# beautifulv0id/Convex-2D-GPU-Collision-Detection

Hardware: AMD Instinct MI355X
Metric: sat_pair_tests_per_s (higher is better)
Workload: dtype f32

## Files before the change

convex-2d-gpu-collision-detection_amd/csrc/c2d_mc_poly.hip:

```cpp
#include <type_traits>

#include "c2d_internal.hpp"
#include "c2d_math.hpp"

#ifdef C2D_MC_STATS
namespace c2d {
__device__ unsigned long long c2d_mc_poly_stats_words[12];
}
#define C2D_MC_STAT(i, v)                                                                                     \
    do {                                                                                                      \
        const unsigned long long v__ = (unsigned long long)(v);                                               \
        if ((threadIdx.x & 63) == 0 && v__) atomicAdd(&c2d::c2d_mc_poly_stats_words[i], v__);                 \
    } while (0)
#endif
#include "c2d_mc_core.hpp"

namespace c2d {

#ifndef C2D_MC_POLY_PLAIN_PAIR_LOOP
#define C2D_MC_POLY_PLAIN_PAIR_LOOP 0
#endif
constexpr int KM = C2D_POLY_KMAX;
#ifndef C2D_MC_POLY_IN_PLACE
#define C2D_MC_POLY_IN_PLACE 48
#endif
#ifndef C2D_MC_POLY_SURV_SLOTS
#define C2D_MC_POLY_SURV_SLOTS ((64 + C2D_MC_POLY_IN_PLACE + 15) / 16 * 16)
#endif
constexpr int kSurvSlots = C2D_MC_POLY_SURV_SLOTS;
static_assert(63 + C2D_MC_POLY_IN_PLACE - 1 < kSurvSlots, "survivor queue too small for a full push");

struct PolyScene {
    float sx, sy, st, sw, sh;
    uint32_t x0;
    bool use_x0;
    int ka, kb;
    C2D_DEV bool tame() const { return use_x0 || x0 != 0u; }
};

struct PolyQueue {
    float4 axis[KM];
    float4 pre[KM];
    float4 ctr[KM];
    float2 rvert[KM];
    float2 overt[KM];
    float4 surv_a[kSurvSlots];
    float2 surv_b[kSurvSlots];
    uint32_t n_surv;
    SampleQueues sq;
};

C2D_DEV float wave_max(float v)
{
#pragma unroll
    for (int off = 32; off > 0; off >>= 1) v = __builtin_fmaxf(v, __shfl_xor(v, off, 64));
    return v;
}

C2D_DEV float lane_pick(const float (&a)[KM], uint32_t l)
{
    float v = a[0];
#pragma unroll
    for (int k = 1; k < KM; k++) v = l == (uint32_t)k ? a[k] : v;
    return v;
}

C2D_DEV PolyScene build_poly_scene(float rvx, float rvy, int ka, float px, float py, float theta, float ovx, float ovy, int kb, const StdDev& sd,
                                   PolyQueue& q)
{
    const uint32_t lane = threadIdx.x & 63, l = lane & 15;
    PolyScene sc;
    sc.sx = sd.x; sc.sy = sd.y; sc.st = sd.theta; sc.sw = sd.width; sc.sh = sd.height;
    sc.ka = ka; sc.kb = kb;
    const float rx0 = __shfl(rvx, 0, 64), ry0 = __shfl(rvy, 0, 64), ox0 = __shfl(ovx, 0, 64), oy0 = __shfl(ovy, 0, 64);
    const float rxl = (int)l < ka ? rvx : rx0, ryl = (int)l < ka ? rvy : ry0;
    const float oxl = (int)l < kb ? ovx : ox0, oyl = (int)l < kb ? ovy : oy0;
    float s, c;
    sincos_(theta, s, c);
    const float wx = dot2(c, rxl, -s, ryl) + px, wy = dot2(s, rxl, c, ryl) + py;
    wave_lds_sync();
    if (lane < KM) {
        q.rvert[l] = make_float2(wx, wy);
        q.overt[l] = make_float2(oxl, oyl);
    }
    if (lane == 0) q.n_surv = 0;
    wave_lds_sync();
    const float2 v1 = q.rvert[(l + 1) & 15];
    const float nx = -(v1.y - wy), ny = v1.x - wx;
    float rmin = 0.0f, rmax = 0.0f, p_first = 0.0f;
#pragma unroll
    for (int k = 0; k < KM; k++) {
        const float2 v = q.rvert[k];
        const float p = nx * v.x + ny * v.y;
        if (k == 0) { rmin = rmax = p_first = p; }
        else { rmin = __builtin_fminf(rmin, p); rmax = __builtin_fmaxf(rmax, p); }
    }
    const float fxm = 1.0f + kNormalMax * __builtin_fabsf(sc.sw), fym = 1.0f + kNormalMax * __builtin_fabsf(sc.sh);
    const float ex = fxm * oxl, ey = fym * oyl;
    const float rho = wave_max(__builtin_sqrtf(ex * ex + ey * ey)) * (1.0f + 0x1p-10f);
    const float D = kNormalMax * (__builtin_fabsf(sc.sx) + __builtin_fabsf(sc.sy));
    const float n2 = __builtin_sqrtf(nx * nx + ny * ny), n1 = __builtin_fabsf(nx) + __builtin_fabsf(ny);
    const float M = (n2 * rho) * (1.0f + 0x1p-10f) + 0x1p-12f * (n1 * (rho + D));
    const float hi = rmax + M, lo = rmin - M;
    float phi = hi + 0x1p-20f * __builtin_fabsf(hi), plo = lo - 0x1p-20f * __builtin_fabsf(lo);
    const bool real_edge = (int)l < ka && n1 > 0.0f;
    if (!real_edge) { phi = __builtin_inff(); plo = -__builtin_inff(); }
    float r0 = 0.0f;
    {
        const float gx = nx * sc.sx, gy = ny * sc.sy;
        const float G = __builtin_sqrtf(gx * gx + gy * gy) * (1.0f + 0x1p-10f);
        const float L = plo > 0.0f ? plo : (phi < 0.0f ? -phi : 0.0f);
        if (real_edge && L > 0.0f && G > 0.0f && L < 1e30f) r0 = L / G;
    }
    const float R0 = wave_max(r0);
    if (lane < KM) {
        q.axis[l] = make_float4(nx, ny, rmin, rmax);
        q.pre[l] = make_float4(plo, phi, p_first, 0.0f);
        q.ctr[l] = make_float4(nx, ny, plo, phi);
    }
    wave_lds_sync();
    auto below = [](float v, float bound) { return __builtin_fabsf(v) < bound; };
    auto length = [](float v) { const float a = __builtin_fabsf(v); return a < 1e8f && (a == 0.0f || a >= 1e-15f); };
    const float rel = 1e4f, ang = 1e15f;
    const bool mine = ((int)l >= ka || (length(rvx) && length(rvy))) && ((int)l >= kb || (length(ovx) && length(ovy)));
    const bool tame = __builtin_amdgcn_ballot_w64(!mine) == 0ull && length(px) && length(py) && below(theta, ang) && length(sd.x) && length(sd.y) &&
                      below(sd.theta, ang) && below(sd.width, rel) && below(sd.height, rel);
    sc.use_x0 = false;
    sc.x0 = 0xffffffffu;
    if (!tame) {
        sc.x0 = 0u;
        return sc;
    }
    radius_word_threshold(R0, sc.x0, sc.use_x0);
    return sc;
}

template <bool NANS>
C2D_DEV float min3_(float a, float b, float c)
{
    if constexpr (NANS) return __builtin_fminf(__builtin_fminf(a, b), c);
    float r;
    asm("v_min3_f32 %0, %1, %2, %3" : "=v"(r) : "v"(a), "v"(b), "v"(c));
    return r;
}
template <bool NANS>
C2D_DEV float max3_(float a, float b, float c)
{
    if constexpr (NANS) return __builtin_fmaxf(__builtin_fmaxf(a, b), c);
    float r;
    asm("v_max3_f32 %0, %1, %2, %3" : "=v"(r) : "v"(a), "v"(b), "v"(c));
    return r;
}

template <int CB>
C2D_DEV void poly_sampled_vertices(const PolyQueue& q, float dx, float dy, float c, float s, float fx, float fy, float (&ox)[CB], float (&oy)[CB])
{
#pragma unroll
    for (int k = 0; k < CB; k++) {
        const float2 b = q.overt[k];
        const float x = fx * b.x, y = fy * b.y;
        ox[k] = dot2(c, x, -s, y) + dx;
        oy[k] = dot2(s, x, c, y) + dy;
    }
}

template <int CB, bool NANS>
C2D_DEV unsigned long long poly_stage_robot(const PolyScene& sc, const PolyQueue& q, const float (&ox)[CB], const float (&oy)[CB], unsigned long long lanes)
{
    unsigned long long sep = 0ull;
    const int ka = sc.ka;
#pragma nounroll
    for (int i = 0; i < ka; i++) {
        const float4 A = q.axis[i];
        float p0 = A.x * ox[0] + A.y * oy[0];
        float omin = p0, omax = p0;
#pragma unroll
        for (int k = 1; k < CB; k++) {
            const float p = A.x * ox[k] + A.y * oy[k];
            omin = __builtin_fminf(omin, p);
            omax = __builtin_fmaxf(omax, p);
        }
        unsigned long long m = __builtin_amdgcn_ballot_w64(A.w < omin) | __builtin_amdgcn_ballot_w64(omax < A.z);
        if constexpr (NANS) m &= __builtin_amdgcn_ballot_w64(first_projections_ordered(q.pre[i].z, p0));
        sep |= m;
    }
    return lanes & ~sep;
}

template <int CB, bool NANS>
C2D_DEV unsigned long long poly_stage_obstacle(const PolyScene& sc, const PolyQueue& q, const float (&ox)[CB], const float (&oy)[CB], unsigned long long lanes)
{
    unsigned long long sep = 0ull;
    const int ka = sc.ka;
    auto group = [&](auto g_const, auto j0_const) {
        constexpr int G = decltype(g_const)::value, j0 = decltype(j0_const)::value;
        float nx[G], ny[G], mn1[G], mx1[G], mn2[G], mx2[G], q0[G], r0[G];
#pragma unroll
        for (int a = 0; a < G; a++) {
            const int j = j0 + a, j1 = (j + 1) % CB;
            nx[a] = -(oy[j1] - oy[j]);
            ny[a] = ox[j1] - ox[j];
            q0[a] = nx[a] * ox[0] + ny[a] * oy[0];
            mn2[a] = mx2[a] = q0[a];
        }
#pragma unroll
        for (int k = 1; k < CB; k++) {
#pragma unroll
            for (int a = 0; a < G; a++) {
                const float p = nx[a] * ox[k] + ny[a] * oy[k];
                mn2[a] = __builtin_fminf(mn2[a], p);
                mx2[a] = __builtin_fmaxf(mx2[a], p);
            }
        }
        const float4* rv2 = reinterpret_cast<const float4*>(q.rvert);
        const int pairs = (ka + 1) >> 1;
#if C2D_MC_POLY_PLAIN_PAIR_LOOP
        float4 cur = rv2[0];
#else
        float4 cur = rv2[0];
        float4 nxt = rv2[pairs > 1 ? 1 : 0];
#endif
#pragma unroll
        for (int a = 0; a < G; a++) {
            r0[a] = nx[a] * cur.x + ny[a] * cur.y;
            const float p1 = nx[a] * cur.z + ny[a] * cur.w;
            mn1[a] = __builtin_fminf(r0[a], p1);
            mx1[a] = __builtin_fmaxf(r0[a], p1);
        }
#pragma nounroll
        for (int j = 1; j < pairs; j++) {
#if C2D_MC_POLY_PLAIN_PAIR_LOOP
            cur = rv2[j];
#else
            cur = nxt;
            nxt = rv2[j + 1 < pairs ? j + 1 : j];
#endif
#pragma unroll
            for (int a = 0; a < G; a++) {
                const float p0 = nx[a] * cur.x + ny[a] * cur.y, p1 = nx[a] * cur.z + ny[a] * cur.w;
                mn1[a] = min3_<NANS>(mn1[a], p0, p1);
                mx1[a] = max3_<NANS>(mx1[a], p0, p1);
            }
        }
#pragma unroll
        for (int a = 0; a < G; a++) {
            unsigned long long m = __builtin_amdgcn_ballot_w64(mx1[a] < mn2[a]) | __builtin_amdgcn_ballot_w64(mx2[a] < mn1[a]);
            if constexpr (NANS) m &= __builtin_amdgcn_ballot_w64(first_projections_ordered(r0[a], q0[a]));
            sep |= m;
        }
    };
    using std::integral_constant;
    if constexpr (CB >= 4) { group(integral_constant<int, 4>{}, integral_constant<int, 0>{}); if ((lanes & ~sep) == 0ull) return 0ull; }
    if constexpr (CB >= 8) { group(integral_constant<int, 4>{}, integral_constant<int, 4>{}); if ((lanes & ~sep) == 0ull) return 0ull; }
    if constexpr (CB >= 12) { group(integral_constant<int, 4>{}, integral_constant<int, 8>{}); if ((lanes & ~sep) == 0ull) return 0ull; }
    if constexpr (CB >= 16) { group(integral_constant<int, 4>{}, integral_constant<int, 12>{}); if ((lanes & ~sep) == 0ull) return 0ull; }
    if constexpr (CB % 4 != 0) group(integral_constant<int, CB % 4>{}, integral_constant<int, CB - CB % 4>{});
    return lanes & ~sep;
}

template <int CB, bool NANS, int STAGE>
C2D_DEV unsigned long long poly_sample_stage(const PolyScene& sc, const PolyQueue& q, float dx, float dy, float c, float s, float fx, float fy,
                                             unsigned long long lanes, bool& final)
{
    float ox[CB], oy[CB];
    poly_sampled_vertices<CB>(q, dx, dy, c, s, fx, fy, ox, oy);
    unsigned long long alive = lanes;
    final = true;
    if constexpr (STAGE != 2) {
        alive = poly_stage_robot<CB, NANS>(sc, q, ox, oy, alive);
        if (alive == 0ull) return 0ull;
    }
    if constexpr (STAGE == 1) {
        if (__popcll(alive) < C2D_MC_POLY_IN_PLACE) { final = false; return alive; }
        C2D_MC_STAT(8, __popcll(alive));
    }
    return poly_stage_obstacle<CB, NANS>(sc, q, ox, oy, alive);
}

template <bool NANS, int STAGE>
C2D_DEV unsigned long long poly_sample_stage_any(const PolyScene& sc, const PolyQueue& q, float dx, float dy, float c, float s, float fx, float fy,
                                                 unsigned long long lanes, bool& final)
{
#ifndef C2D_MC_POLY_EVEN_SLOTS
#define C2D_MC_POLY_EVEN_SLOTS 0
#endif
#define C2D_POLY_STAGE(CB) return poly_sample_stage<CB, NANS, STAGE>(sc, q, dx, dy, c, s, fx, fy, lanes, final)
    if constexpr (NANS || C2D_MC_POLY_EVEN_SLOTS) {
        switch ((sc.kb + 1) >> 1) {
        case 1: C2D_POLY_STAGE(2);
        case 2: C2D_POLY_STAGE(4);
        case 3: C2D_POLY_STAGE(6);
        case 4: C2D_POLY_STAGE(8);
        case 5: C2D_POLY_STAGE(10);
        case 6: C2D_POLY_STAGE(12);
        case 7: C2D_POLY_STAGE(14);
        default: C2D_POLY_STAGE(16);
        }
    } else {
        switch (sc.kb) {
        case 1: C2D_POLY_STAGE(1);
        case 2: C2D_POLY_STAGE(2);
        case 3: C2D_POLY_STAGE(3);
        case 4: C2D_POLY_STAGE(4);
        case 5: C2D_POLY_STAGE(5);
        case 6: C2D_POLY_STAGE(6);
        case 7: C2D_POLY_STAGE(7);
        case 8: C2D_POLY_STAGE(8);
        case 9: C2D_POLY_STAGE(9);
        case 10: C2D_POLY_STAGE(10);
        case 11: C2D_POLY_STAGE(11);
        case 12: C2D_POLY_STAGE(12);
        case 13: C2D_POLY_STAGE(13);
        case 14: C2D_POLY_STAGE(14);
        case 15: C2D_POLY_STAGE(15);
        default: C2D_POLY_STAGE(16);
        }
    }
#undef C2D_POLY_STAGE
}

C2D_DEV void poly_sample_shape(const PolyScene& sc, uint32_t radius_word, uint32_t angle_word, uint64_t seed, uint64_t scene_id, uint64_t sample, float& c,
                               float& s, float& fx, float& fy)
{
    float n2, n3;
    box_muller(radius_word, angle_word, n2, n3);
    const float dt = n2 * sc.st;
    const float dw = n3 * sc.sw;
    float dh = 0.0f;
    if (sc.sh != 0.0f) {
        const U4 b = philox_draw_block(seed, scene_id, sample >> 2, 4u + ((uint32_t)(sample >> 1) & 1u));
        const bool odd = (sample & 1) != 0;
        float n4, unused;
        box_muller(odd ? b.z : b.x, odd ? b.w : b.y, n4, unused);
        dh = n4 * sc.sh;
    }
    fx = 1.0f + dw;
    fy = 1.0f + dh;
    sincos_(dt, s, c);
}

struct PolyPolicy {
    using Scene = PolyScene;
    using Queue = PolyQueue;
    static C2D_DEV bool centre_pretest(const Scene& sc, const Queue& q, float dx, float dy, unsigned long long& miss_m)
    {
        bool miss = false;
#pragma nounroll
        for (int i = 0; i < sc.ka; i++) {
            const float4 A = q.ctr[i];
            const float t = fma_(A.x, dx, A.y * dy);
            miss |= (t > A.w) | (t < A.z);
        }
        miss_m = __builtin_amdgcn_ballot_w64(miss);
        return miss;
    }
    static C2D_DEV uint32_t evaluate_survivors(const Scene& sc, Queue& q, uint32_t& n, uint32_t take)
    {
        const uint32_t lane = threadIdx.x & 63;
        wave_lds_sync();
        const unsigned long long live_m = take >= 64 ? ~0ull : (1ull << take) - 1;
        const uint32_t src = n - take + (lane < take ? lane : 0);
        const float4 a = q.surv_a[src];
        const float2 b = q.surv_b[src];
        wave_lds_sync();
        n -= take;
        bool final;
        C2D_MC_STAT(9, take);
        return (uint32_t)__popcll(poly_sample_stage_any<false, 2>(sc, q, a.x, a.y, a.z, a.w, b.x, b.y, live_m, final));
    }
    static C2D_DEV uint32_t evaluate(const Scene& sc, Queue& q, uint32_t w2r, uint32_t w2a, float dx, float dy, uint64_t seed, uint64_t scene_id, uint64_t sample,
                                     unsigned long long live_m)
    {
        float c, s, fx, fy;
        poly_sample_shape(sc, w2r, w2a, seed, scene_id, sample, c, s, fx, fy);
        bool final;
        C2D_MC_STAT(5, __popcll(live_m));
        const unsigned long long alive = poly_sample_stage_any<false, 1>(sc, q, dx, dy, c, s, fx, fy, live_m, final);
        if (final) return (uint32_t)__popcll(alive);
        C2D_MC_STAT(6, __popcll(alive));
        uint32_t n = q.n_surv;
        if ((alive >> (threadIdx.x & 63)) & 1ull) {
            const uint32_t slot = n + __builtin_amdgcn_mbcnt_hi((uint32_t)(alive >> 32), __builtin_amdgcn_mbcnt_lo((uint32_t)alive, 0u));
            q.surv_a[slot] = make_float4(dx, dy, c, s);
            q.surv_b[slot] = make_float2(fx, fy);
        }
        n += (uint32_t)__popcll(alive);
        uint32_t hits = 0;
        if (n >= 64) hits = evaluate_survivors(sc, q, n, 64);
        wave_lds_sync();
        if ((threadIdx.x & 63) == 0) q.n_surv = n;
        wave_lds_sync();
        return hits;
    }
    static C2D_DEV uint32_t finish(const Scene& sc, Queue& q)
    {
        uint32_t n = q.n_surv;
        if (n == 0) return 0u;
        uint32_t hits = 0;
        while (n) hits += evaluate_survivors(sc, q, n, n < 64 ? n : 64u);
        wave_lds_sync();
        if ((threadIdx.x & 63) == 0) q.n_surv = 0;
        wave_lds_sync();
        return hits;
    }
    static C2D_DEV uint32_t plain(const Scene& sc, uint64_t seed, uint64_t scene_id, uint64_t begin, uint32_t count, const Queue& q)
    {
        const uint32_t lane = threadIdx.x & 63;
        uint32_t hits = 0;
#pragma nounroll
        for (uint32_t i = 0; i < count; i += 64) {
            const uint32_t left = count - i;
            const unsigned long long live_m = left >= 64 ? ~0ull : (1ull << left) - 1;
            const uint64_t sm = begin + i + lane;
            const uint32_t j = (uint32_t)sm & 3u;
            const U4 b0 = philox_draw_block(seed, scene_id, sm >> 2, 0), b1 = philox_draw_block(seed, scene_id, sm >> 2, 1);
            const U4 b2 = philox_draw_block(seed, scene_id, sm >> 2, 2u + (j >> 1));
            float dx, dy, c, s, fx, fy;
            sample_centre(sc, u4_word(b0, (int)j), u4_word(b1, (int)j), dx, dy);
            poly_sample_shape(sc, (j & 1u) ? b2.z : b2.x, (j & 1u) ? b2.w : b2.y, seed, scene_id, sm, c, s, fx, fy);
            bool final;
            hits += (uint32_t)__popcll(poly_sample_stage_any<true, 0>(sc, q, dx, dy, c, s, fx, fy, live_m, final));
        }
        return hits;
    }
};

struct PolyPairArgs {
    c2d_polygon robot, obstacle;
    float px, py, theta;
    StdDev sd;
    uint64_t seed, scene_id, sample_begin, n_samples;
    uint32_t chunk;
};

#ifndef C2D_MC_POLY_WAVES
#define C2D_MC_POLY_WAVES 5
#endif
#ifdef C2D_MC_CLOCK
C2D_MC_CLOCK_WORDS(c2d_mc_clock_poly_pair);
C2D_MC_CLOCK_WORDS(c2d_mc_clock_poly);
#endif
__global__ __launch_bounds__(kMcBlock, C2D_MC_POLY_WAVES) void mc_poly_pair_kernel(PolyPairArgs A, unsigned long long* __restrict__ d_hits)
{
    __shared__ PolyQueue s_queue[kWavesPerBlock];
    const uint32_t wave = __builtin_amdgcn_readfirstlane(threadIdx.x >> 6);
    const uint32_t l = threadIdx.x & 15;
    const PolyScene sc = build_poly_scene(lane_pick(A.robot.x, l), lane_pick(A.robot.y, l), (int)A.robot.k, A.px, A.py, A.theta, lane_pick(A.obstacle.x, l),
                                          lane_pick(A.obstacle.y, l), (int)A.obstacle.k, A.sd, s_queue[wave]);
    const uint64_t n_chunks = (A.n_samples + A.chunk - 1) / A.chunk;
    unsigned long long total = 0;
    C2D_MC_CLOCK_START();
    for (uint64_t ch = (uint64_t)blockIdx.x * kWavesPerBlock + wave; ch < n_chunks; ch += (uint64_t)gridDim.x * kWavesPerBlock) {
        const uint64_t off = ch * A.chunk;
        const uint64_t left = A.n_samples - off;
        const uint32_t count = left < A.chunk ? (uint32_t)left : A.chunk;
        total += wave_count_hits<PolyPolicy>(sc, A.seed, A.scene_id, A.sample_begin + off, count, s_queue[wave]);
    }
    C2D_MC_CLOCK_STOP(c2d_mc_clock_poly_pair);
    if ((threadIdx.x & 63) == 0 && total) atomicAdd(d_hits, total);
}

struct PolyScenesArgs {
    const StdDev* std_devs;
    const PositionWithVarAndPoseIdx* scenes;
    AdaptiveState* state;
    uint32_t* lists[2];
    uint32_t num_std_devs;
    uint64_t seed, scene_id_base;
    ScheduleArgs sched;
    uint32_t* hits;
    uint32_t burst_steps;
    uint32_t n_bins;
    float bins[16], acc[16];
    uint32_t* n_used;
    PoseCPVarAndPoseIdx* rows;
    const c2d_poly_pose* poly_poses;
    uint32_t num_poly_poses;
    c2d_polygon robot;
    uint32_t* async_err;
};

struct PolyBuilder {
    using Args = PolyScenesArgs;
    using Policy = PolyPolicy;
#ifdef C2D_MC_CLOCK
    static C2D_DEV unsigned long long* clock_words() { return c2d_mc_clock_poly; }
#endif
    static C2D_DEV PolyScene scene(const Args& A, const PositionWithVarAndPoseIdx& row, PolyQueue& q)
    {
        uint32_t pi = (uint32_t)(int)row.pose_idx, vi = (uint32_t)(int)row.var_idx;
        pi = pi < A.num_poly_poses ? pi : A.num_poly_poses - 1;
        vi = vi < A.num_std_devs ? vi : A.num_std_devs - 1;
        const c2d_poly_pose* pp = A.poly_poses + pi;
        const uint32_t l = threadIdx.x & 15;
        const float theta = pp->theta, ovx = pp->obstacle.x[l], ovy = pp->obstacle.y[l];
        uint32_t kb = pp->obstacle.k, ka = A.robot.k;
        if (kb < 1 || kb > (uint32_t)KM) {
            if ((threadIdx.x & 63) == 0) __hip_atomic_fetch_or(A.async_err, C2D_ASYNC_ERR_POLY_K, __ATOMIC_RELAXED, __HIP_MEMORY_SCOPE_SYSTEM);
            kb = kb < 1 ? 1u : (uint32_t)KM;
        }
        ka = ka < 1 ? 1u : (ka > (uint32_t)KM ? (uint32_t)KM : ka);
        return build_poly_scene(lane_pick(A.robot.x, l), lane_pick(A.robot.y, l), (int)ka, row.x, row.y, theta, ovx, ovy, (int)kb, A.std_devs[vi], q);
    }
};

template <bool BURST>
__global__ __launch_bounds__(kMcBlock, C2D_MC_POLY_WAVES) void mc_poly_scenes_advance_kernel(PolyScenesArgs A) { mc_scenes_advance_body<BURST, PolyBuilder>(A); }

}

using namespace c2d;

namespace {

const char* polygon_fault(const c2d_polygon* p)
{
    if (!p) return "NULL polygon";
    if (p->k < 1 || p->k > (uint32_t)C2D_POLY_KMAX) return "polygon vertex count outside 1..C2D_POLY_KMAX";
    return nullptr;
}

c2d_polygon tidy(const c2d_polygon& p)
{
    c2d_polygon o = p;
    for (uint32_t k = p.k; k < (uint32_t)C2D_POLY_KMAX; k++) o.x[k] = o.y[k] = 0.0f;
    return o;
}

}

extern "C" {

int c2d_mc_poly_pair(c2d_ctx* ctx, const c2d_polygon* robot, const Position* pos, float robot_theta, const c2d_polygon* obstacle, const StdDev* std_dev,
                     uint64_t seed, uint64_t scene_id, uint64_t sample_begin, uint64_t n_samples, unsigned long long* d_hits, c2d_stream stream)
{
    if (!ctx) return C2D_ERR_INVALID_ARG;
    if (!robot || !pos || !obstacle || !std_dev || !d_hits) return fail_arg(ctx, "c2d_mc_poly_pair: NULL argument");
    if (const char* f = polygon_fault(robot)) return fail_arg(ctx, (std::string("c2d_mc_poly_pair: robot: ") + f).c_str());
    if (const char* f = polygon_fault(obstacle)) return fail_arg(ctx, (std::string("c2d_mc_poly_pair: obstacle: ") + f).c_str());
    if (n_samples == 0) return C2D_OK;
    if (sample_begin + n_samples < sample_begin || sample_begin + n_samples > (1ull << 62))
        return fail_arg(ctx, "c2d_mc_poly_pair: sample range overflows the 2^62-sample stream");
    PolyPairArgs A;
    A.robot = tidy(*robot); A.obstacle = tidy(*obstacle);
    A.px = pos->x; A.py = pos->y; A.theta = robot_theta; A.sd = *std_dev;
    A.seed = seed; A.scene_id = scene_id; A.sample_begin = sample_begin; A.n_samples = n_samples;
    const uint64_t target_waves = (uint64_t)ctx->prop.multiProcessorCount * 32;
    uint64_t chunk = (n_samples + target_waves - 1) / target_waves;
    chunk = ((chunk + 255) / 256) * 256;
    if (chunk < 256) chunk = 256;
    if (chunk > 8192) chunk = 8192;
    A.chunk = (uint32_t)chunk;
    const uint64_t n_chunks = (n_samples + chunk - 1) / chunk;
    uint64_t blocks = (n_chunks + kWavesPerBlock - 1) / kWavesPerBlock;
    const uint64_t max_blocks = (uint64_t)ctx->prop.multiProcessorCount * 256 / kWavesPerBlock;
    if (blocks > max_blocks) blocks = max_blocks;
    DeviceGuard g(ctx->device);
    hipLaunchKernelGGL(mc_poly_pair_kernel, dim3((unsigned)blocks), dim3(kMcBlock), 0, (hipStream_t)stream, A, d_hits);
    C2D_LAUNCH_CHECK(ctx);
    return C2D_OK;
}

int c2d_mc_poly_scenes(c2d_ctx* ctx, const c2d_mc_poly_scenes_args* a, c2d_stream stream)
{
    if (!ctx) return C2D_ERR_INVALID_ARG;
    if (!a) return fail_arg(ctx, "c2d_mc_poly_scenes: NULL args");
    const c2d_mc_scenes_args* b = &a->base;
    if (b->n_scenes != 0) {
        const char* why = nullptr;
        if (!a->d_poly_poses) why = "c2d_mc_poly_scenes: NULL argument";
        else if (a->num_poly_poses == 0) why = "c2d_mc_poly_scenes: empty pose / std_dev table";
        else if (polygon_fault(a->robot)) why = "c2d_mc_poly_scenes: robot: NULL or vertex count outside 1..C2D_POLY_KMAX";
        if (why) {
            if (b->total_samples) *b->total_samples = 0;
            if (b->iterations) *b->iterations = 0;
            return fail_arg(ctx, why);
        }
    }
    PolyScenesArgs A;
    A.poly_poses = a->d_poly_poses; A.num_poly_poses = a->num_poly_poses;
    if (a->robot) A.robot = tidy(*a->robot);
    A.async_err = ctx->d_async_err;
    return run_adaptive(ctx, b, stream, A, [](bool burst, unsigned blocks, const PolyScenesArgs& args, hipStream_t s) {
        if (burst) hipLaunchKernelGGL(mc_poly_scenes_advance_kernel<true>, dim3(blocks), dim3(kMcBlock), 0, s, args);
        else hipLaunchKernelGGL(mc_poly_scenes_advance_kernel<false>, dim3(blocks), dim3(kMcBlock), 0, s, args);
    }, "c2d_mc_poly_scenes");
}

#ifdef C2D_MC_STATS
int c2d_debug_mc_poly_stats(c2d_ctx* ctx, unsigned long long out[12], int reset)
{
    if (!ctx || !out) return C2D_ERR_INVALID_ARG;
    DeviceGuard g(ctx->device);
    C2D_HIP(ctx, hipDeviceSynchronize());
    C2D_HIP(ctx, hipMemcpyFromSymbol(out, HIP_SYMBOL(c2d_mc_poly_stats_words), 12 * sizeof(unsigned long long)));
    if (reset) {
        const unsigned long long zero[12] = {};
        C2D_HIP(ctx, hipMemcpyToSymbol(HIP_SYMBOL(c2d_mc_poly_stats_words), zero, sizeof zero));
    }
    return C2D_OK;
}
#endif

#ifdef C2D_MC_CLOCK
int c2d_debug_mc_poly_clock(c2d_ctx* ctx, int which, unsigned long long out[4], int reset)
{
    if (!ctx || !out || which < 0 || which > 1) return C2D_ERR_INVALID_ARG;
    DeviceGuard g(ctx->device);
    C2D_HIP(ctx, hipDeviceSynchronize());
    const unsigned long long zero[4] = {};
    if (which == 0) {
        C2D_HIP(ctx, hipMemcpyFromSymbol(out, HIP_SYMBOL(c2d_mc_clock_poly_pair), 4 * sizeof(unsigned long long)));
        if (reset) C2D_HIP(ctx, hipMemcpyToSymbol(HIP_SYMBOL(c2d_mc_clock_poly_pair), zero, sizeof zero));
    } else {
        C2D_HIP(ctx, hipMemcpyFromSymbol(out, HIP_SYMBOL(c2d_mc_clock_poly), 4 * sizeof(unsigned long long)));
        if (reset) C2D_HIP(ctx, hipMemcpyToSymbol(HIP_SYMBOL(c2d_mc_clock_poly), zero, sizeof zero));
    }
    return C2D_OK;
}
#endif

}
```

profiles/counts.py:

```python
#!/usr/bin/env python3
from __future__ import annotations

import json
import os
import re
import sys

HERE = os.path.dirname(os.path.abspath(__file__))
OUT = os.path.join(HERE, "measured_counts.json")

ENTRIES = {
    "sat_rect_verts.config2": (["c2d::sat_rect_verts_kernel<4, 64>"], "pairs", 10_000_000, "valu_instr_per_pair"),
    "sat_rect_verts_mask.config2": (["c2d::sat_rect_verts_mask4_kernel"], "pairs", 10_000_000, "valu_instr_per_pair"),
    "sat_rect_pose.config2": (["c2d::sat_rect_pose_kernel<4, 64>"], "pairs", 10_000_000, "valu_instr_per_pair"),
    "sat_poly.config5": (["c2d::sat_poly_kernel<16, 5, true>"], "pairs", 10_000_000, "valu_instr_per_pair"),
    "sat_poly4.small_polygons": (["c2d::sat_poly4_kernel"], "pairs", 10_000_000, "valu_instr_per_pair"),
    "sat_poly_binned.config5": (["c2d::sat_poly_binned_kernel"], "pairs", 10_000_000, "valu_instr_per_pair"),
    "mc_pair.config3": (["c2d::mc_pair_kernel"], "samples", 100_000_000, "valu_instr_per_sample"),
    "mc_poly_pair.bench": (["c2d::mc_poly_pair_kernel"], "samples", 100_000_000, "valu_instr_per_sample"),
    "mc_scenes.config4": (["c2d::mc_scenes_advance_kernel<true>", "c2d::mc_scenes_advance_kernel<false>"], "drawn_samples", None, "valu_instr_per_sample"),
    "mc_poly_scenes.bench": (["c2d::mc_poly_scenes_advance_kernel<true>", "c2d::mc_poly_scenes_advance_kernel<false>"], "drawn_samples", "poly", "valu_instr_per_sample"),
}


CARRIED = ("evaluated_fraction", "evaluated_source", "held_clock_ghz", "held_clock_source")


def read_sq(path):
    out = {}
    for ln in open(path):
        m = re.match(r"(.{42}) (\S+)\s+n=\s*(\d+) mean=\s*([\d.]+)", ln)
        if m:
            out.setdefault(m.group(1).strip(), {})[m.group(2)] = (int(m.group(3)), float(m.group(4)))
    return out


def build(tag: str) -> dict:
    sq_path, hbm_path, bench_path = (os.path.join(HERE, f"{tag}_{n}") for n in ("pmc_sq.txt", "pmc_hbm.json", "bench.json"))
    sq = read_sq(sq_path)
    hbm = json.load(open(hbm_path)) if os.path.exists(hbm_path) else {}
    issue_path = os.path.join(HERE, f"{tag}_valu_issue.json")
    issue = json.load(open(issue_path)).get("entries", {}) if os.path.exists(issue_path) else {}
    bench = json.loads(open(bench_path).read().strip().splitlines()[-1]) if os.path.exists(bench_path) else {}
    res = {"_doc": "GENERATED by profiles/counts.py from the digests named in each entry's `source` (do not edit): VALU instructions per unit "
                   "(SQ_INSTS_VALU x 64 lanes / units) and HBM traffic per launch (2 x FETCH_SIZE + WRITE_SIZE) of the kernels on the "
                   "bench.py workloads. bench.py attaches them to its rooflines only when the workload matches; they are recorded values, "
                   "not measured in the bench run.", "_tag": tag}
    for name, (kernels, unit_key, units, per_key) in ENTRIES.items():
        found = [k for k in kernels if any(s.startswith(k[:40]) for s in sq)]
        if len(found) != len(kernels):
            continue
        wave_instr = 0.0
        for k in kernels:
            key = next(s for s in sq if s.startswith(k[:40]))
            n, mean = sq[key]["SQ_INSTS_VALU"]
            wave_instr += mean * (n if units is None or units == "poly" else 1)
        e = {}
        if units is None:
            sc = bench.get("scenes") or {}
            if not sc:
                continue
            drawn = sc["mean_samples_per_point"] * sc["data_points_per_gpu"]
            e["data_points"] = sc["data_points_per_gpu"]
            e["max_samples"] = sc["max_samples"]
            e["drawn_samples"] = drawn
            e[per_key] = round(wave_instr * 64 / drawn, 1)
        elif units == "poly":
            sc = (bench.get("mc_poly") or {}).get("scenes") or {}
            if not sc:
                continue
            drawn = sc["mean_samples_per_scene"] * sc["scenes_per_gpu"]
            e["scenes"] = sc["scenes_per_gpu"]
            e["max_samples"] = sc["max_samples"]
            e["drawn_samples"] = drawn
            e[per_key] = round(wave_instr * 64 / (2 * drawn), 1)
        else:
            e[unit_key] = units
            e[per_key] = round(wave_instr * 64 / units, 1)
        srcs = [f"profiles/{tag}_pmc_sq.txt"]
        hk = next((h for h in hbm if h.startswith(kernels[0][:40])), None) if units not in (None, "poly") else None
        if hk:
            e["hbm_bytes_per_launch"] = int(round(hbm[hk]["hbm_bytes_per_launch_corrected"]))
            srcs.append(f"profiles/{tag}_pmc_hbm.json")
        if units is None or units == "poly":
            srcs.append(f"profiles/{tag}_bench.json")
        if issue.get(name, {}).get("mix_ticks_per_wave_instr"):
            e["issue_ticks_per_wave_instr"] = issue[name]["mix_ticks_per_wave_instr"]
            srcs.append(f"profiles/{tag}_valu_issue.json")
        e["source"] = ", ".join(srcs)
        res[name] = e
    return res


def carry_over(new: dict, old: dict) -> dict:
    for k, v in old.items():
        if k in new and isinstance(v, dict):
            for f in CARRIED:
                if f in v and f not in new[k]:
                    new[k][f] = v[f]
    return new


def verify() -> list[str]:
    cur = json.load(open(OUT))
    tag = cur.get("_tag")
    if not tag:
        return ["measured_counts.json has no _tag: regenerate it with `python profiles/counts.py write <tag>`"]
    fresh = build(tag)
    bad = []
    for k, v in cur.items():
        if k.startswith("_"):
            continue
        if k not in fresh:
            bad.append(f"{k}: not derivable from the digests of tag {tag}")
            continue
        for f, val in v.items():
            if f in CARRIED:
                continue
            if fresh[k].get(f) != val:
                bad.append(f"{k}.{f}: recorded {val!r}, the digests give {fresh[k].get(f)!r}")
    return bad


if __name__ == "__main__":
    if len(sys.argv) >= 3 and sys.argv[1] == "write":
        old = json.load(open(OUT)) if os.path.exists(OUT) else {}
        json.dump(carry_over(build(sys.argv[2]), old), open(OUT, "w"), indent=1)
        print("wrote", OUT)
    elif len(sys.argv) >= 2 and sys.argv[1] == "verify":
        problems = verify()
        for p in problems:
            print("MISMATCH", p)
        sys.exit(1 if problems else 0)
    else:
        raise SystemExit(__doc__)
```

Baseline: 96.74 billion.

## Certify polygon overlaps early via convex-interior test in the robot stage

Setup now checks whether the robot polygon is consistently wound (CCW or CW), orients its edge axes to match, and stores a per-edge inner threshold. It also rotates the obstacle vertices so the deepest vertex comes first. In the first Monte Carlo stage, a sample with a sampled obstacle vertex inside every robot half-plane is counted as a certain hit, so it skips the survivor queue and the obstacle-axis stage. This costs extra setup work, extra ballots per robot axis, and relies on conservative tolerances for correctness; counts.py gains per-entry digest files.

```diff
diff --git a/convex-2d-gpu-collision-detection_amd/csrc/c2d_mc_poly.hip b/convex-2d-gpu-collision-detection_amd/csrc/c2d_mc_poly.hip
--- a/convex-2d-gpu-collision-detection_amd/csrc/c2d_mc_poly.hip
+++ b/convex-2d-gpu-collision-detection_amd/csrc/c2d_mc_poly.hip
@@ -35,6 +35,7 @@
     uint32_t x0;
     bool use_x0;
     int ka, kb;
+    bool certify;
     C2D_DEV bool tame() const { return use_x0 || x0 != 0u; }
 };
 
@@ -113,23 +114,63 @@
         if (real_edge && L > 0.0f && G > 0.0f && L < 1e30f) r0 = L / G;
     }
     const float R0 = wave_max(r0);
-    if (lane < KM) {
-        q.axis[l] = make_float4(nx, ny, rmin, rmax);
-        q.pre[l] = make_float4(plo, phi, p_first, 0.0f);
-        q.ctr[l] = make_float4(nx, ny, plo, phi);
-    }
-    wave_lds_sync();
     auto below = [](float v, float bound) { return __builtin_fabsf(v) < bound; };
     auto length = [](float v) { const float a = __builtin_fabsf(v); return a < 1e8f && (a == 0.0f || a >= 1e-15f); };
     const float rel = 1e4f, ang = 1e15f;
     const bool mine = ((int)l >= ka || (length(rvx) && length(rvy))) && ((int)l >= kb || (length(ovx) && length(ovy)));
     const bool tame = __builtin_amdgcn_ballot_w64(!mine) == 0ull && length(px) && length(py) && below(theta, ang) && length(sd.x) && length(sd.y) &&
                       below(sd.theta, ang) && below(sd.width, rel) && below(sd.height, rel);
+    const float Cr = wave_max(__builtin_fmaxf(__builtin_fabsf(wx), __builtin_fabsf(wy)));
+    const float Cc = __builtin_fmaxf(Cr,
+                                     rho + kNormalMax * __builtin_fmaxf(__builtin_fabsf(sc.sx), __builtin_fabsf(sc.sy)));
+    const uint32_t nxt = (int)l + 1 < ka ? l + 1 : 0u;
+    const float nnx = __shfl(nx, (int)nxt, 64), nny = __shfl(ny, (int)nxt, 64);
+    const float pe0 = nx * wx + ny * wy, pe1 = nx * v1.x + ny * v1.y;
+    const float tau = 0x1p-20f * (n1 * Cr);
+    const bool at_min = __builtin_fmaxf(pe0, pe1) <= rmin + tau, at_max = __builtin_fminf(pe0, pe1) >= rmax - tau;
+    const float cu = nx * nny, cv = ny * nnx;
+    const float cr = cu - cv, cmag = 0x1p-12f * (__builtin_fabsf(cu) + __builtin_fabsf(cv));
+    const bool mine_ccw = (int)l >= ka || (n1 > 0.0f && at_min && cr > cmag);
+    const bool mine_cw = (int)l >= ka || (n1 > 0.0f && at_max && -cr > cmag);
+    const bool ccw = __builtin_amdgcn_ballot_w64(!mine_ccw) == 0ull, cw = __builtin_amdgcn_ballot_w64(!mine_cw) == 0ull;
+    float tin = ((ccw ? rmin : -rmax) + (0x1p-10f * (n1 * Cc) + 0x1p-120f));
+    tin = tin + 0x1p-20f * __builtin_fabsf(tin);
+    const bool t_finite = __builtin_amdgcn_ballot_w64((int)l < ka && !(__builtin_fabsf(tin) < __builtin_inff())) == 0ull;
+    sc.certify = tame && ka >= 3 && (ccw || cw) && t_finite;
+#ifdef C2D_MC_POLY_NO_CERTIFY
+    sc.certify = false;
+#endif
+    const bool flip = sc.certify && !ccw;
+    const float ax = flip ? -nx : nx, ay = flip ? -ny : ny, amin = flip ? -rmax : rmin, amax = flip ? -rmin : rmax;
+    if (lane < KM) {
+        q.axis[l] = make_float4(ax, ay, amin, amax);
+        q.pre[l] = make_float4(plo, phi, p_first, tin);
+        q.ctr[l] = make_float4(nx, ny, plo, phi);
+    }
+    wave_lds_sync();
+    C2D_MC_STAT(11, !sc.certify);
     sc.use_x0 = false;
     sc.x0 = 0xffffffffu;
     if (!tame) {
         sc.x0 = 0u;
         return sc;
+    }
+    if (sc.certify) {
+        float depth = __builtin_inff();
+#pragma nounroll
+        for (int i = 0; i < ka; i++) {
+            const float4 A = q.axis[i];
+            depth = __builtin_fminf(depth, ((A.x * oxl + A.y * oyl) - A.z) / (__builtin_fabsf(A.x) + __builtin_fabsf(A.y)));
+        }
+        if ((int)l >= kb) depth = -__builtin_inff();
+        const float deepest = wave_max(depth);
+        const uint32_t best = (uint32_t)__builtin_ctzll(__builtin_amdgcn_ballot_w64(depth == deepest && (int)l < kb)) & 15u;
+        uint32_t src = l + best;
+        src = src >= (uint32_t)kb ? src - (uint32_t)kb : src;
+        src = (int)l < kb ? src : best;
+        const float rox = __shfl(oxl, (int)src, 64), roy = __shfl(oyl, (int)src, 64);
+        if (lane < KM) q.overt[l] = make_float2(rox, roy);
+        wave_lds_sync();
     }
     radius_word_threshold(R0, sc.x0, sc.use_x0);
     return sc;
@@ -185,6 +226,35 @@
         sep |= m;
     }
     return lanes & ~sep;
+}
+
+template <int CB>
+C2D_DEV unsigned long long poly_stage_robot_certify(const PolyScene& sc, const PolyQueue& q, const float (&ox)[CB], const float (&oy)[CB],
+                                                    unsigned long long lanes, unsigned long long& certain)
+{
+    unsigned long long sep = 0ull, in0 = ~0ull, in1 = CB >= 2 ? ~0ull : 0ull, in2 = CB >= 3 ? ~0ull : 0ull;
+    const int ka = sc.ka;
+#pragma nounroll
+    for (int i = 0; i < ka; i++) {
+        const float4 A = q.axis[i];
+        const float t = q.pre[i].w;
+        float p[CB];
+#pragma unroll
+        for (int k = 0; k < CB; k++) p[k] = A.x * ox[k] + A.y * oy[k];
+        float omin = p[0], omax = p[0];
+#pragma unroll
+        for (int k = 1; k < CB; k++) {
+            omin = __builtin_fminf(omin, p[k]);
+            omax = __builtin_fmaxf(omax, p[k]);
+        }
+        sep |= __builtin_amdgcn_ballot_w64(A.w < omin) | __builtin_amdgcn_ballot_w64(omax < A.z);
+        in0 &= __builtin_amdgcn_ballot_w64(p[0] >= t);
+        if constexpr (CB >= 2) in1 &= __builtin_amdgcn_ballot_w64(p[1] >= t);
+        if constexpr (CB >= 3) in2 &= __builtin_amdgcn_ballot_w64(p[CB - 1] >= t);
+    }
+    const unsigned long long alive = lanes & ~sep;
+    certain = alive & (in0 | in1 | in2);
+    return alive;
 }
 
 template <int CB, bool NANS>
@@ -260,13 +330,25 @@
 
 template <int CB, bool NANS, int STAGE>
 C2D_DEV unsigned long long poly_sample_stage(const PolyScene& sc, const PolyQueue& q, float dx, float dy, float c, float s, float fx, float fy,
-                                             unsigned long long lanes, bool& final)
+                                             unsigned long long lanes, bool& final, uint32_t& certain)
 {
     float ox[CB], oy[CB];
     poly_sampled_vertices<CB>(q, dx, dy, c, s, fx, fy, ox, oy);
     unsigned long long alive = lanes;
     final = true;
-    if constexpr (STAGE != 2) {
+    certain = 0;
+    if constexpr (STAGE == 1) {
+        if (sc.certify) {
+            unsigned long long cert_m;
+            alive = poly_stage_robot_certify<CB>(sc, q, ox, oy, alive, cert_m);
+            certain = (uint32_t)__popcll(cert_m);
+            C2D_MC_STAT(10, certain);
+            alive &= ~cert_m;
+        } else {
+            alive = poly_stage_robot<CB, NANS>(sc, q, ox, oy, alive);
+        }
+        if (alive == 0ull) return 0ull;
+    } else if constexpr (STAGE != 2) {
         alive = poly_stage_robot<CB, NANS>(sc, q, ox, oy, alive);
         if (alive == 0ull) return 0ull;
     }
@@ -279,12 +361,12 @@
 
 template <bool NANS, int STAGE>
 C2D_DEV unsigned long long poly_sample_stage_any(const PolyScene& sc, const PolyQueue& q, float dx, float dy, float c, float s, float fx, float fy,
-                                                 unsigned long long lanes, bool& final)
+                                                 unsigned long long lanes, bool& final, uint32_t& certain)
 {
 #ifndef C2D_MC_POLY_EVEN_SLOTS
 #define C2D_MC_POLY_EVEN_SLOTS 0
 #endif
-#define C2D_POLY_STAGE(CB) return poly_sample_stage<CB, NANS, STAGE>(sc, q, dx, dy, c, s, fx, fy, lanes, final)
+#define C2D_POLY_STAGE(CB) return poly_sample_stage<CB, NANS, STAGE>(sc, q, dx, dy, c, s, fx, fy, lanes, final, certain)
     if constexpr (NANS || C2D_MC_POLY_EVEN_SLOTS) {
         switch ((sc.kb + 1) >> 1) {
         case 1: C2D_POLY_STAGE(2);
@@ -365,8 +447,9 @@
         wave_lds_sync();
         n -= take;
         bool final;
+        uint32_t certain;
         C2D_MC_STAT(9, take);
-        return (uint32_t)__popcll(poly_sample_stage_any<false, 2>(sc, q, a.x, a.y, a.z, a.w, b.x, b.y, live_m, final));
+        return (uint32_t)__popcll(poly_sample_stage_any<false, 2>(sc, q, a.x, a.y, a.z, a.w, b.x, b.y, live_m, final, certain));
     }
     static C2D_DEV uint32_t evaluate(const Scene& sc, Queue& q, uint32_t w2r, uint32_t w2a, float dx, float dy, uint64_t seed, uint64_t scene_id, uint64_t sample,
                                      unsigned long long live_m)
@@ -375,8 +458,9 @@
         poly_sample_shape(sc, w2r, w2a, seed, scene_id, sample, c, s, fx, fy);
         bool final;
         C2D_MC_STAT(5, __popcll(live_m));
-        const unsigned long long alive = poly_sample_stage_any<false, 1>(sc, q, dx, dy, c, s, fx, fy, live_m, final);
-        if (final) return (uint32_t)__popcll(alive);
+        uint32_t hits;
+        const unsigned long long alive = poly_sample_stage_any<false, 1>(sc, q, dx, dy, c, s, fx, fy, live_m, final, hits);
+        if (final) return hits + (uint32_t)__popcll(alive);
         C2D_MC_STAT(6, __popcll(alive));
         uint32_t n = q.n_surv;
         if ((alive >> (threadIdx.x & 63)) & 1ull) {
@@ -385,8 +469,7 @@
             q.surv_b[slot] = make_float2(fx, fy);
         }
         n += (uint32_t)__popcll(alive);
-        uint32_t hits = 0;
-        if (n >= 64) hits = evaluate_survivors(sc, q, n, 64);
+        if (n >= 64) hits += evaluate_survivors(sc, q, n, 64);
         wave_lds_sync();
         if ((threadIdx.x & 63) == 0) q.n_surv = n;
         wave_lds_sync();
@@ -419,7 +502,8 @@
             sample_centre(sc, u4_word(b0, (int)j), u4_word(b1, (int)j), dx, dy);
             poly_sample_shape(sc, (j & 1u) ? b2.z : b2.x, (j & 1u) ? b2.w : b2.y, seed, scene_id, sm, c, s, fx, fy);
             bool final;
-            hits += (uint32_t)__popcll(poly_sample_stage_any<true, 0>(sc, q, dx, dy, c, s, fx, fy, live_m, final));
+            uint32_t certain;
+            hits += (uint32_t)__popcll(poly_sample_stage_any<true, 0>(sc, q, dx, dy, c, s, fx, fy, live_m, final, certain));
         }
         return hits;
     }
diff --git a/profiles/counts.py b/profiles/counts.py
--- a/profiles/counts.py
+++ b/profiles/counts.py
@@ -20,6 +20,12 @@
     "mc_poly_pair.bench": (["c2d::mc_poly_pair_kernel"], "samples", 100_000_000, "valu_instr_per_sample"),
     "mc_scenes.config4": (["c2d::mc_scenes_advance_kernel<true>", "c2d::mc_scenes_advance_kernel<false>"], "drawn_samples", None, "valu_instr_per_sample"),
     "mc_poly_scenes.bench": (["c2d::mc_poly_scenes_advance_kernel<true>", "c2d::mc_poly_scenes_advance_kernel<false>"], "drawn_samples", "poly", "valu_instr_per_sample"),
+}
+
+
+ENTRY_DIGESTS = {
+    "mc_poly_pair.bench": "mc_poly_r22",
+    "mc_poly_scenes.bench": "mc_poly_r22",
 }
 
 
@@ -46,7 +52,12 @@
                    "(SQ_INSTS_VALU x 64 lanes / units) and HBM traffic per launch (2 x FETCH_SIZE + WRITE_SIZE) of the kernels on the "
                    "bench.py workloads. bench.py attaches them to its rooflines only when the workload matches; they are recorded values, "
                    "not measured in the bench run.", "_tag": tag}
+    tag_sq = sq
     for name, (kernels, unit_key, units, per_key) in ENTRIES.items():
+        sq, sq_src = tag_sq, f"profiles/{tag}_pmc_sq.txt"
+        own = os.path.join(HERE, f"{tag}_{ENTRY_DIGESTS[name]}_pmc_sq.txt") if name in ENTRY_DIGESTS else None
+        if own and os.path.exists(own):
+            sq, sq_src = read_sq(own), f"profiles/{os.path.basename(own)}"
         found = [k for k in kernels if any(s.startswith(k[:40]) for s in sq)]
         if len(found) != len(kernels):
             continue
@@ -77,7 +88,7 @@
         else:
             e[unit_key] = units
             e[per_key] = round(wave_instr * 64 / units, 1)
-        srcs = [f"profiles/{tag}_pmc_sq.txt"]
+        srcs = [sq_src]
         hk = next((h for h in hbm if h.startswith(kernels[0][:40])), None) if units not in (None, "poly") else None
         if hk:
             e["hbm_bytes_per_launch"] = int(round(hbm[hk]["hbm_bytes_per_launch_corrected"]))
```

Result: no change. 96.88 billion, median of 3 (+0.1%).
